# carlamb/MovieRecommender-TF-TRT

Measured on NVIDIA B200. Metric: ncf_train_samples_per_sec, higher is better.
Workload: dtype f32

## Files before the change

movierecommender-tf-trt_b200/csrc/api.cu:

```cuda
#include <math.h>
#include <stdarg.h>
#include <stdlib.h>
#include <string.h>

#include <vector>

#include "launchers.h"
#include "neumf_tile.cuh"

namespace mr {

static thread_local char g_err[512] = "";

void set_error(const char* fmt, ...) {
  va_list ap;
  va_start(ap, fmt);
  vsnprintf(g_err, sizeof(g_err), fmt, ap);
  va_end(ap);
}

int cuda_fail(cudaError_t e, const char* what) {
  set_error("CUDA error in %s: %s", what, cudaGetErrorString(e));
  return MR_ERR_CUDA;
}
// ... 27 lines not shown
};
static thread_local Profiler g_prof;
constexpr size_t kMaxProfEvents = 1 << 16;

void count_launch() { g_prof.launches += 1; }

void prof_mark(int phase, cudaStream_t st) {
  Profiler& p = g_prof;
  if (!p.on) return;
  if (p.used >= kMaxProfEvents) {
    p.overflow = true;
    return;
  }
  if (p.used == p.events.size()) {
    cudaEvent_t e;
    if (cudaEventCreate(&e) != cudaSuccess) {
      cudaGetLastError();
      p.overflow = true;
      return;
    }
    p.events.push_back(e);
    p.phase.push_back(-1);
  }
  cudaEventRecord(p.events[p.used], st);
  p.phase[p.used] = phase;
  p.used += 1;
}

struct SideStream {
  int dev = -1;
  cudaStream_t stream = nullptr;
  cudaEvent_t fork = nullptr, join = nullptr;
  cudaEvent_t fork2 = nullptr, join2 = nullptr;
};
static thread_local SideStream g_side;

static SideStream* side_stream() {
  int dev = 0;
  if (cudaGetDevice(&dev) != cudaSuccess) {
    cudaGetLastError();
    return nullptr;
  }
  SideStream& s = g_side;
  if (s.dev != dev) {
    s = SideStream{};
    if (cudaStreamCreateWithFlags(&s.stream, cudaStreamNonBlocking) != cudaSuccess ||
        cudaEventCreateWithFlags(&s.fork, cudaEventDisableTiming) != cudaSuccess ||
        cudaEventCreateWithFlags(&s.join, cudaEventDisableTiming) != cudaSuccess ||
        cudaEventCreateWithFlags(&s.fork2, cudaEventDisableTiming) != cudaSuccess ||
        cudaEventCreateWithFlags(&s.join2, cudaEventDisableTiming) != cudaSuccess) {
      cudaGetLastError();
      s = SideStream{};
      return nullptr;
    }
    s.dev = dev;
  }
  return &s;
}

__global__ void flag_to_float_kernel(const int32_t* flags, float* out) {
  *out = (float)((flags[0] ? 1 : 0) | (flags[1] ? 2 : 0));
}

static int bits_for(int64_t n) {
  int b = 1;
  while (b < 31 && ((int64_t)1 << b) < n) ++b;
  return b;
}

static int sort_row_ids(const int32_t* ids, int64_t n, int32_t num_rows, int32_t* sorted_keys, int32_t* sorted_index,
                        void* ws, size_t ws_bytes, cudaStream_t st) {
  return launch_sort_pairs(ids, n, bits_for((int64_t)num_rows + 1), sorted_keys, sorted_index, ws, ws_bytes, st,
                           num_rows);
}

static int check_model(const MrModel* m) {
  MR_REQUIRE(m != nullptr, "model is NULL");
  MR_REQUIRE(m->n_layers >= 1 && m->n_layers <= MR_MAX_LAYERS, "n_layers=%d out of [1,%d]", m->n_layers, MR_MAX_LAYERS);
  MR_REQUIRE(m->L[0] >= 2, "layers_sizes[0]=%d must be >= 2", m->L[0]);
  for (int l = 0; l < m->n_layers; ++l)
    MR_REQUIRE(m->L[l] >= 1 && m->L[l] <= MR_MAX_WIDTH, "layers_sizes[%d]=%d out of [1,%d]", l, m->L[l], MR_MAX_WIDTH);
  MR_REQUIRE(m->mf_dim >= 0 && m->mf_dim <= MR_MAX_WIDTH, "mf_dim=%d out of range", m->mf_dim);
  MR_REQUIRE(m->num_users > 0 && m->num_items > 0, "num_users/num_items must be > 0");
// ... 279 lines not shown
  a.K = m.L[0] - d_u;
  a.rows = m.num_items;
  a.row0 = 0;
  a.epilogue = TC_EPI_BIAS_RELU;
  a.linear = true;
  a.out = t.Pi;
  return launch_tc_dense(a, st);
}

static int tc_project_users(const MrModel& m, const TcWs& t, cudaStream_t st) {
  TcDenseArgs a{};
  a.a_dense = m.user_mlp;
  a.b_packed = t.pack_fu;
  a.N = m.L[1];
  a.K = m.L[0] / 2;
  a.rows = m.num_users;
  a.row0 = 0;
  a.epilogue = TC_EPI_BIAS_RELU;
  a.bias = m.b[1];
  a.linear = true;
  a.out = t.Pu;
  return launch_tc_dense(a, st);
}

struct TrainWs {
  int32_t* flags;
  float* wt;
  float* dense_partial;
  int64_t dense_stride;
  float* loss_partial;
  float* probs;
  float* stage_u;
  float* stage_i;
  int32_t* sorted_keys;
  int32_t* sorted_index;
  int32_t* sorted_keys_i;
  int32_t* sorted_index_i;
  void* sort_ws;
  size_t sort_ws_bytes;
  void* seg_ws;
  size_t seg_ws_bytes;
  void* seg_ws_u;
  size_t seg_ws_u_bytes;
  void* tc_ws;
  size_t tc_ws_bytes;
  void* small_ws;
  size_t small_ws_bytes;
  int32_t* pos;
  float* rank_partials;
  int32_t* group_users;
  size_t total;
};

static TrainWs carve_train(const MrModel& m, int64_t B, void* ws) {
  TrainWs t;
  Carver cv(ws);
  const int d_u = m.L[0] / 2, d_i = m.L[0] - d_u;
  const int cap = max_tile_ctas();
  t.flags = cv.take<int32_t>(64);
  t.wt = cv.take<float>(m.dense_count);
  t.dense_stride = (m.dense_count + 3) & ~(int64_t)3;
  t.dense_partial = cv.take<float>((size_t)cap * t.dense_stride);
  t.loss_partial = cv.take<float>(cap);
  t.probs = cv.take<float>(B);
  t.stage_u = cv.take<float>((size_t)B * (d_u + m.mf_dim));
  t.stage_i = cv.take<float>((size_t)B * (d_i + m.mf_dim));
  t.sorted_keys = cv.take<int32_t>(B);
  t.sorted_index = cv.take<int32_t>(B);
  t.sorted_keys_i = cv.take<int32_t>(B);
  t.sorted_index_i = cv.take<int32_t>(B);
  t.sort_ws_bytes = sort_workspace_bytes(B);
  t.sort_ws = cv.take<char>(t.sort_ws_bytes);
  t.seg_ws_bytes = segreduce_workspace_bytes(B, (d_u > d_i ? d_u : d_i) + m.mf_dim);
  t.seg_ws = cv.take<char>(t.seg_ws_bytes);
  t.seg_ws_u_bytes = segreduce_workspace_bytes(B / 2 + 1, d_u + m.mf_dim);
  t.seg_ws_u = cv.take<char>(t.seg_ws_u_bytes);
  t.pos = cv.take<int32_t>(B);
  t.rank_partials = cv.take<float>(rank_partials_count(B));
  t.group_users = cv.take<int32_t>(B / 2 + 1);
  t.tc_ws_bytes = tc_eligible(m) ? carve_tc(m, true, B, nullptr).total : 0;
  t.tc_ws = cv.take<char>(t.tc_ws_bytes);
  t.small_ws_bytes = (!tc_eligible(m) && small_tower_supported(m, 5)) ? carve_small(m, nullptr).total : 0;
  t.small_ws = cv.take<char>(t.small_ws_bytes);
  t.total = cv.off;
  return t;
}

static float adam_lr_t(const MrOptState& o, int64_t t) {
  return (float)((double)o.lr * sqrt(1.0 - pow((double)o.beta_2, (double)t)) / (1.0 - pow((double)o.beta_1, (double)t)));
}

static int check_opt(const MrModel& m, const MrOptState* o, const MrGrads* g) {
  MR_REQUIRE(o != nullptr && g != nullptr, "opt/grads is NULL");
  MR_REQUIRE(o->optimizer == MR_OPT_ADAM || o->optimizer == MR_OPT_SGD, "unknown optimizer %d", o->optimizer);
  MR_REQUIRE(o->table_mode == MR_TABLES_DENSE || o->table_mode == MR_TABLES_SPARSE, "unknown table_mode %d", o->table_mode);
  MR_REQUIRE(g->dense != nullptr, "grads.dense is NULL");
  if (o->optimizer == MR_OPT_ADAM) {
    MR_REQUIRE(o->m_dense && o->v_dense && o->m_user_mlp && o->v_user_mlp && o->m_item_mlp && o->v_item_mlp,
               "Adam state pointers are NULL");
// ... 360 lines not shown
      if (rc == MR_OK) rc = launch_pack_weights(Wu, d_u, m.L[1], 1, tw.pack_bu, st);
      if (rc == MR_OK) rc = launch_pack_weights(Wi, d_i, m.L[1], 1, tw.pack_bi, st);
      if (rc != MR_OK) return rc;
    }
    if (proj) {
      prof_mark(MR_PHASE_TC_DENSE_FWD, st);
      rc = tc_project_items(m, tw, st);
      if (rc == MR_OK && uproj) rc = tc_project_users(m, tw, st);
      if (rc != MR_OK) return rc;
    }
    int fused_grid = 0;
    if (fused) {
      prof_mark(MR_PHASE_FUSED_TILE, st);
      FusedTrainArgs fa{};
      fa.Pi = tw.Pi;
      fa.Pu = tw.Pu;
      fa.user_gmf = m.user_gmf;
      fa.item_gmf = m.item_gmf;
      fa.users = users;
      fa.items = items;
      fa.labels = labels;
      fa.num_users = m.num_users;
      fa.num_items = m.num_items;
      fa.rows = B;
      fa.group = group;
      fa.W2 = m.W[2];
      fa.w2_image = tw.w2_image;
      fa.b2 = m.b[2];
      fa.w_out = m.w_out;
      fa.b_out = m.b_out;
      fa.inv_batch = inv_global_batch;
      fa.probs = t.probs;
      fa.stage_i = t.stage_i;
      fa.stage_u = t.stage_u;
      fa.si = d_i + f;
      fa.su = d_u + f;
      fa.partial = t.dense_partial;
      fa.partial_stride = t.dense_stride;
      fa.off_w2 = m.W[2] - m.dense;
      fa.off_b2 = m.b[2] - m.dense;
      fa.off_wout = m.w_out - m.dense;
      fa.off_bout = m.b_out - m.dense;
      fa.loss_partial = t.loss_partial;
      fa.flags = t.flags;
      rc = launch_fused_train(fa, st, &fused_grid);
      if (rc != MR_OK) return rc;
    }
    const int64_t sb = tc_sub_batch(B);
    for (int64_t r0 = 0; r0 < B && !fused; r0 += sb) {
      const int64_t r1 = r0 + sb < B ? r0 + sb : B;
      prof_mark(MR_PHASE_TC_DENSE_FWD, st);
      rc = tc_forward_rows(m, tw, users, items, 1, r0, r1, st, gdiv);
      if (rc != MR_OK) return rc;
      prof_mark(MR_PHASE_HEAD, st);
      HeadArgs h{};
      h.model = model;
      h.h_last = tw.H[n - 1];
      h.users = users;
      h.items = items;
      h.labels = labels;
      h.rows = r1 - r0;
      h.row0 = r0;
      h.user_div = 1;
      h.group = gdiv;
      h.inv_batch = inv_global_batch;
      h.probs = t.probs;
      h.dz_last = tw.dZ[n - 1];
      h.stage_u = t.stage_u;
// ... 135 lines not shown
          a.si = d_i + f;
        }
        rc = launch_tc_dense(a, st);
        if (rc != MR_OK) return rc;
      }
    }
    if (proj) {
      if (side != nullptr) MR_CUDA(cudaStreamWaitEvent(st, side->join, 0));
      RowUpdate ui{};
      ui.mode = MR_TABLES_DENSE;
      ui.optimizer = opt->optimizer;
      ui.d0 = m.L[1];
      ui.d1 = f;
      ui.num_rows = m.num_items;
      ui.g0 = tw.Si;
      ui.g1 = grads->item_gmf;
      cudaStream_t su_st = st;
      if (uproj && side != nullptr) {
        MR_CUDA(cudaEventRecord(side->fork2, st));
        MR_CUDA(cudaStreamWaitEvent(side->stream, side->fork2, 0));
        su_st = side->stream;
      }
      if (uproj && su_st != st) {
        RowUpdate uu{};
        uu.mode = MR_TABLES_DENSE;
        uu.optimizer = opt->optimizer;
        uu.d0 = m.L[1];
        uu.d1 = f;
        uu.num_rows = m.num_users;
        uu.g0 = tw.Su;
        uu.g1 = grads->user_gmf;
        rc = launch_segreduce(t.sorted_keys, t.sorted_index, n_user_rows, t.stage_u, uu, t.seg_ws_u, t.seg_ws_u_bytes, su_st);
        if (rc != MR_OK) return rc;
        if (grads->user_gmf_ready != nullptr) {
          MR_CUDA(cudaEventRecord((cudaEvent_t)grads->user_gmf_ready, su_st));
          user_gmf_event_recorded = true;
        }
        TcDenseArgs bu{};
        bu.a_dense = tw.Su;
        bu.b_packed = tw.pack_bu;
        bu.N = d_u;
        bu.K = m.L[1];
        bu.rows = m.num_users;
        bu.row0 = 0;
        bu.epilogue = TC_EPI_BIAS_RELU;
        bu.linear = true;
        bu.out = grads->user_mlp;
        rc = launch_tc_dense(bu, su_st);
        if (rc != MR_OK) return rc;
        TcWgradArgs wu{};
        wu.a_dense = m.user_mlp;
        wu.z = tw.Su;
        wu.Fa = d_u;
        wu.Fb = m.L[1];
        wu.rows = m.num_users;
        wu.row0 = 0;
        wu.dw_partial = t.dense_partial + (m.W[1] - m.dense);
        wu.db_partial = t.dense_partial + (m.b[1] - m.dense);
        wu.partial_stride = t.dense_stride;
        rc = launch_tc_wgrad(wu, su_st);
        if (rc != MR_OK) return rc;
        if (grads->user_tables_ready != nullptr) {
          MR_CUDA(cudaEventRecord((cudaEvent_t)grads->user_tables_ready, su_st));
          user_event_recorded = true;
        }
        MR_CUDA(cudaEventRecord(side->join2, su_st));
      }
      prof_mark(MR_PHASE_SEGREDUCE, st);
      rc = launch_segreduce(t.sorted_keys_i, t.sorted_index_i, B, t.stage_i, ui, t.seg_ws, t.seg_ws_bytes, st);
      if (rc != MR_OK) return rc;
      if (uproj && su_st == st) {
        RowUpdate uu{};
        uu.mode = MR_TABLES_DENSE;
        uu.optimizer = opt->optimizer;
        uu.d0 = m.L[1];
        uu.d1 = f;
        uu.num_rows = m.num_users;
        uu.g0 = tw.Su;
        uu.g1 = grads->user_gmf;
        prof_mark(MR_PHASE_SEGREDUCE, st);
        rc = launch_segreduce(t.sorted_keys, t.sorted_index, n_user_rows, t.stage_u, uu, t.seg_ws, t.seg_ws_bytes, st);
        if (rc != MR_OK) return rc;
      }
      prof_mark(MR_PHASE_TC_DENSE_BWD, st);
      TcDenseArgs bi{};
      bi.a_dense = tw.Si;
      bi.b_packed = tw.pack_bi;
      bi.N = d_i;
      bi.K = m.L[1];
      bi.rows = m.num_items;
      bi.row0 = 0;
      bi.epilogue = TC_EPI_BIAS_RELU;
      bi.linear = true;
      bi.out = grads->item_mlp;
      rc = launch_tc_dense(bi, st);
      if (rc != MR_OK) return rc;
      prof_mark(MR_PHASE_TC_WGRAD, st);
      TcWgradArgs wi{};
      wi.a_dense = m.item_mlp;
      wi.z = tw.Si;
      wi.Fa = d_i;
      wi.Fb = m.L[1];
      wi.rows = m.num_items;
// ... 668 lines not shown
```

movierecommender-tf-trt_b200/csrc/launchers.h:

```cpp
#pragma once

#include "common.cuh"

namespace mr {

struct TileLaunch {
  const MrModel* model;
  bool train;
  const float* wt;
  const int32_t* users;
  const int32_t* items;
  const float* labels;
  int64_t B;
  int32_t user_div;
  float inv_batch;
  float* logits;
  float* probs;
  float* loss_partial;
  float* dense_partial;
  int64_t dense_stride;
  float* stage_u;
  float* stage_i;
  int32_t* flags;
};
int max_tile_ctas();
int choose_tile_rows(const MrModel& m, bool train);
int launch_neumf_tiles(const TileLaunch& a, cudaStream_t st, int* grid_out);
int launch_transpose_kernels(const MrModel& m, float* wt, cudaStream_t st);
int launch_dense_reduce(const MrModel& m, const float* partial, int64_t stride, int grid_ctas, float* out,
                        cudaStream_t st, bool with_l2 = true);
int launch_sum_partials(const float* partial, int n, float* out, cudaStream_t st);
int launch_l2_penalty(const float* x, int64_t n, float coef, float* out, cudaStream_t st);

int launch_gather_rows(const float* table, int64_t rows, int dim, const int32_t* idx, int64_t n, float* out,
                       cudaStream_t st);

size_t sort_workspace_bytes(int64_t n);
int launch_sort_pairs(const int32_t* keys, int64_t n, int key_bits, int32_t* out_keys, int32_t* out_index,
                      void* ws, size_t ws_bytes, cudaStream_t st, int32_t num_rows = -1);

struct RowUpdate {
  int mode;
  int optimizer;
  float lr_t, beta_1, beta_2, epsilon, lr;
  int d0, d1;
  int num_rows;
  float *p0, *m0, *v0, *g0;
  float *p1, *m1, *v1, *g1;
};
size_t segreduce_workspace_bytes(int64_t n, int ld);
int launch_segreduce(const int32_t* sorted_keys, const int32_t* sorted_index, int64_t n, const float* staged,
                     const RowUpdate& u, void* ws, size_t ws_bytes, cudaStream_t st);

constexpr int kMaxOptRegions = 5;
struct OptRegions {
  float* p[kMaxOptRegions];
  const float* g[kMaxOptRegions];
  float* m[kMaxOptRegions];
  float* v[kMaxOptRegions];
  int64_t n[kMaxOptRegions];
  float l2[kMaxOptRegions];
  int count;
  int block_start[kMaxOptRegions + 1];
};
int launch_optimizer_regions(OptRegions r, int optimizer, float lr_t, float beta_1, float beta_2, float epsilon,
                             cudaStream_t st);
int launch_optimizer_flat(float* p, const float* g, float* m, float* v, int64_t n, int optimizer, float lr_t,
                          float beta_1, float beta_2, float epsilon, float l2, cudaStream_t st);

size_t rank_partials_count(int64_t G);
int launch_rank_scores(const float* scores, int64_t G, int group, int k, const int32_t* label_col, int32_t* rank,
                       int32_t* pos, float* sums, float* partials, cudaStream_t st, const float* labels = nullptr);

struct TopkArgs {
  const float* scores;
  int64_t U, u0;
  int32_t N, k;
  const int32_t* excl_ids;
  int32_t excl_rows;
  const int64_t* excl_rowptr;
  const int32_t* excl_items;
  const int32_t* targets;
  const int32_t* users;
  int32_t num_users;
  int32_t* top_items;
// ... 139 lines not shown
int launch_group_heads(const int32_t* ids, int64_t groups, int group, int32_t* out, cudaStream_t st);
int launch_check_grouped(const int32_t* ids, int64_t n, int group, int32_t* flag, cudaStream_t st);

size_t split_workspace_bytes(int64_t n);
int launch_split_last_two(const int32_t* users, int64_t n, int32_t num_users, int32_t* order, int32_t* part,
                          int32_t* flag, void* ws, size_t ws_bytes, cudaStream_t st);
size_t remap_workspace_bytes(int64_t n);
int launch_remap_ids(const int32_t* ids, int64_t n, int32_t limit, int32_t* dense, int32_t* unique, int64_t* num_unique,
                     int32_t* flag, void* ws, size_t ws_bytes, cudaStream_t st);
size_t user_csr_workspace_bytes(int64_t n);
int launch_build_user_csr(const int32_t* users, const int32_t* items, int64_t n, int32_t num_users, int32_t num_items,
                          int64_t* rowptr, int32_t* csr_items, int32_t* flag, void* ws, size_t ws_bytes,
                          cudaStream_t st);

struct FusedTrainArgs {
  const float* Pi;
  const float* Pu;
  const float* user_gmf;
  const float* item_gmf;
  const int32_t* users;
  const int32_t* items;
  const float* labels;
  int32_t num_users, num_items;
  int64_t rows;
  int32_t group;
  const float* W2;
  uint16_t* w2_image;
  const float* b2;
  const float* w_out;
  const float* b_out;
  float inv_batch;
  float* probs;
  float* stage_i;
  float* stage_u;
  int32_t si, su;
  float* partial;
  int64_t partial_stride;
  int64_t off_w2, off_b2, off_wout, off_bout;
  float* loss_partial;
  int32_t* flags;
};
bool fused_train_supported(const MrModel& m, int group);
size_t fused_w2_image_bytes();
int launch_fused_train(const FusedTrainArgs& a, cudaStream_t st, int* grid_out);
int launch_bf16x3_selftest(const float* A, const float* B, float* D, int N, int K, int a_mn, int b_mn, cudaStream_t st);

int launch_tc_rate(int N, int iters, int nbuf, int flags, int writers, int write_iters, long long* out, int grid,
                   cudaStream_t st);
int launch_tc_probe(const float* raw_a, int n_words, int start_off, int lbo, int sbo, int a_mn, float* D,
                    cudaStream_t st);
int launch_tc_selftest(const float* A, const float* B, float* D, int N, int K, int a_mn, int b_mn, int three_x,
                       cudaStream_t st);

}
```

movierecommender-tf-trt_b200/csrc/segreduce.cu:

```cuda
#include "launchers.h"

namespace mr {

constexpr int kSkip = -1;
constexpr int kPastEnd = -2;
constexpr int kNoNeighbour = -3;
constexpr int kBatch = 8;
constexpr int kBatchUpper = 16;

__device__ __forceinline__ void apply_row_value(const RowUpdate& u, int row, int c, float g) {
  float *p, *m, *v, *gt;
  int d, col;
  if (c < u.d0) {
    p = u.p0; m = u.m0; v = u.v0; gt = u.g0; d = u.d0; col = c;
  } else {
    p = u.p1; m = u.m1; v = u.v1; gt = u.g1; d = u.d1; col = c - u.d0;
  }
  const size_t at = (size_t)row * d + col;
  if (u.mode == MR_TABLES_DENSE) {
    gt[at] = g;
  } else if (u.optimizer == MR_OPT_ADAM) {
    const float mn = u.beta_1 * m[at] + (1.f - u.beta_1) * g;
    const float vn = u.beta_2 * v[at] + (1.f - u.beta_2) * g * g;
    m[at] = mn;
// ... 14 lines not shown
  }
  const size_t at = (size_t)row * d + col;
  if ((d & 3) != 0) {
    apply_row_value(u, row, c, g.x);
    apply_row_value(u, row, c + 1, g.y);
    apply_row_value(u, row, c + 2, g.z);
    apply_row_value(u, row, c + 3, g.w);
    return;
  }
  if (u.mode == MR_TABLES_DENSE) {
    *reinterpret_cast<float4*>(gt + at) = g;
  } else if (u.optimizer == MR_OPT_ADAM) {
    const float4 m0 = *reinterpret_cast<const float4*>(m + at), v0 = *reinterpret_cast<const float4*>(v + at);
    float4 pw = *reinterpret_cast<const float4*>(p + at);
    float4 mn, vn;
    mn.x = u.beta_1 * m0.x + (1.f - u.beta_1) * g.x; vn.x = u.beta_2 * v0.x + (1.f - u.beta_2) * g.x * g.x;
    mn.y = u.beta_1 * m0.y + (1.f - u.beta_1) * g.y; vn.y = u.beta_2 * v0.y + (1.f - u.beta_2) * g.y * g.y;
    mn.z = u.beta_1 * m0.z + (1.f - u.beta_1) * g.z; vn.z = u.beta_2 * v0.z + (1.f - u.beta_2) * g.z * g.z;
    mn.w = u.beta_1 * m0.w + (1.f - u.beta_1) * g.w; vn.w = u.beta_2 * v0.w + (1.f - u.beta_2) * g.w * g.w;
    pw.x = pw.x - u.lr_t * mn.x / (sqrtf(vn.x) + u.epsilon);
    pw.y = pw.y - u.lr_t * mn.y / (sqrtf(vn.y) + u.epsilon);
    pw.z = pw.z - u.lr_t * mn.z / (sqrtf(vn.z) + u.epsilon);
    pw.w = pw.w - u.lr_t * mn.w / (sqrtf(vn.w) + u.epsilon);
    *reinterpret_cast<float4*>(m + at) = mn;
    *reinterpret_cast<float4*>(v + at) = vn;
    *reinterpret_cast<float4*>(p + at) = pw;
  } else {
    float4 pw = *reinterpret_cast<const float4*>(p + at);
    pw.x -= u.lr * g.x; pw.y -= u.lr * g.y; pw.z -= u.lr * g.z; pw.w -= u.lr * g.w;
    *reinterpret_cast<float4*>(p + at) = pw;
  }
}

struct ChunkInfo {
  int nvalid;
  bool first_inc;
  bool last_inc;
  int64_t chunk;
  int ld;
  float* out_rows;
};

template <bool VEC>
__device__ __forceinline__ void flush_run(const RowUpdate& u, const ChunkInfo& ci, int key, int s, int t, int c,
                                          bool on, float4 acc) {
  if (key == kSkip || !on || (unsigned)key >= (unsigned)u.num_rows) return;
  const bool inc_first = (s == 0) && ci.first_inc;
  const bool inc_last = (t == ci.nvalid) && ci.last_inc;
  if (!inc_first && !inc_last) {
    if (VEC) apply_row_value4(u, key, c, acc);
    else apply_row_value(u, key, c, acc.x);
    return;
  }
  float* slot0 = ci.out_rows + (size_t)(2 * ci.chunk) * ci.ld + c;
  float* slot1 = slot0 + ci.ld;
  if (VEC) {
    if (inc_first) {
      *reinterpret_cast<float4*>(slot0) = acc;
      if (inc_last) *reinterpret_cast<float4*>(slot1) = make_float4(0.f, 0.f, 0.f, 0.f);
    } else {
      *reinterpret_cast<float4*>(slot1) = acc;
    }
  } else {
    if (inc_first) {
      *slot0 = acc.x;
      if (inc_last) *slot1 = 0.f;
    } else {
      *slot1 = acc.x;
    }
  }
}

template <bool INDIRECT, bool VEC, int KB>
__global__ void __launch_bounds__(256) segreduce_level_kernel(const int32_t* __restrict__ keys,
                                                              const int32_t* __restrict__ index, int64_t n,
                                                              const float* __restrict__ rows, int32_t* __restrict__ out_keys,
                                                              float* __restrict__ out_rows, const RowUpdate u) {
  const int lane = threadIdx.x & 31;
  const int64_t chunk = ((int64_t)blockIdx.x * blockDim.x + threadIdx.x) >> 5;
  const int64_t base = chunk * 32;
  if (base >= n) return;
  const int ld = u.d0 + u.d1;
  const int64_t e = base + lane;
  const int key = e < n ? __ldg(keys + e) : kPastEnd;
  const int64_t src = e < n ? (INDIRECT ? (int64_t)__ldg(index + e) : e) : 0;
  const bool ok = e < n && key != kSkip;
  const int kprev = base > 0 ? __ldg(keys + base - 1) : kNoNeighbour;
  const int knext = base + 32 < n ? __ldg(keys + base + 32) : kNoNeighbour;
  int kup = __shfl_up_sync(0xffffffffu, key, 1);
  const unsigned starts = __ballot_sync(0xffffffffu, e < n && (lane == 0 || key != kup));

  ChunkInfo ci;
  ci.nvalid = (int)min((int64_t)32, n - base);
  const int key0 = __shfl_sync(0xffffffffu, key, 0);
  const int keyl = __shfl_sync(0xffffffffu, key, ci.nvalid - 1);
  ci.first_inc = key0 != kSkip && kprev == key0;
  ci.last_inc = ci.nvalid == 32 && keyl != kSkip && knext == keyl;
  ci.chunk = chunk;
  ci.ld = ld;
  ci.out_rows = out_rows;
  if (out_keys != nullptr && lane == 0 && blockIdx.y == 0) {
    out_keys[2 * chunk] = ci.first_inc ? key0 : kSkip;
    out_keys[2 * chunk + 1] = ci.last_inc ? keyl : kSkip;
  }

  constexpr int W = VEC ? 4 : 1;
  for (int cb = blockIdx.y * 32 * W; cb < ld; cb += gridDim.y * 32 * W) {
    const int c = cb + lane * W;
    const bool on = c < ld;
    float4 acc = make_float4(0.f, 0.f, 0.f, 0.f);
    int run_key = key0, run_start = 0;
    for (int j0 = 0; j0 < ci.nvalid; j0 += KB) {
      float4 v[KB];
#pragma unroll
      for (int q = 0; q < KB; ++q) {
        const int j = j0 + q;
        const int64_t sj = __shfl_sync(0xffffffffu, src, j);
        const bool okj = __shfl_sync(0xffffffffu, (int)ok, j) != 0;
        v[q] = make_float4(0.f, 0.f, 0.f, 0.f);
        if (okj && on) {
          if (VEC) v[q] = ld_stream4(rows + (size_t)sj * ld + c);
          else v[q].x = __ldg(rows + (size_t)sj * ld + c);
        }
      }
#pragma unroll
      for (int q = 0; q < KB; ++q) {
        const int j = j0 + q;
        if (j < ci.nvalid) {
          if (j > 0 && ((starts >> j) & 1u)) {
            flush_run<VEC>(u, ci, run_key, run_start, j, c, on, acc);
            acc = make_float4(0.f, 0.f, 0.f, 0.f);
            run_start = j;
            run_key = __shfl_sync(0xffffffffu, key, j);
          }
          acc.x += v[q].x;
          if (VEC) {
            acc.y += v[q].y;
            acc.z += v[q].z;
            acc.w += v[q].w;
          }
        }
      }
    }
    flush_run<VEC>(u, ci, run_key, run_start, ci.nvalid, c, on, acc);
  }
}

static int64_t level_entries(int64_t n) { return 2 * ((n + 31) / 32); }

size_t segreduce_workspace_bytes(int64_t n, int ld) {
  const int64_t n1 = level_entries(n < 1 ? 1 : n), n2 = level_entries(n1);
  return align_up((size_t)n1 * 4, 256) + align_up((size_t)n2 * 4, 256) + align_up((size_t)n1 * ld * 4, 256) +
         align_up((size_t)n2 * ld * 4, 256);
}

int launch_segreduce(const int32_t* sorted_keys, const int32_t* sorted_index, int64_t n, const float* staged,
                     const RowUpdate& u, void* ws, size_t ws_bytes, cudaStream_t st) {
  if (n == 0) return MR_OK;
  const int ld = u.d0 + u.d1;
  if (ws_bytes < segreduce_workspace_bytes(n, ld)) {
    set_error("segreduce workspace too small: %zu < %zu", ws_bytes, segreduce_workspace_bytes(n, ld));
    return MR_ERR_WORKSPACE;
  }
  const int64_t n1 = level_entries(n), n2 = level_entries(n1);
  Carver cv(ws);
  int32_t* kbuf[2] = {cv.take<int32_t>(n1), cv.take<int32_t>(n2)};
  float* rbuf[2] = {cv.take<float>((size_t)n1 * ld), cv.take<float>((size_t)n2 * ld)};
  uintptr_t align = reinterpret_cast<uintptr_t>(staged);
  for (const float* q : {u.p0, u.m0, u.v0, u.g0, u.p1, u.m1, u.v1, u.g1}) align |= reinterpret_cast<uintptr_t>(q);
  const bool vec = (ld & 3) == 0 && (u.d0 & 3) == 0 && (align & 15) == 0;

  const int32_t* keys = sorted_keys;
  const float* rows = staged;
  int64_t cur = n;
  for (int level = 0;; ++level) {
    const int64_t nchunks = (cur + 31) / 32;
    const bool last = nchunks == 1;
    int32_t* ok = last ? nullptr : kbuf[level & 1];
    float* orows = last ? nullptr : rbuf[level & 1];
    const unsigned blocks = (unsigned)((nchunks + 7) / 8);
    if (level == 0) {
      if (vec) segreduce_level_kernel<true, true, kBatch><<<blocks, 256, 0, st>>>(keys, sorted_index, cur, rows, ok, orows, u);
      else segreduce_level_kernel<true, false, kBatch><<<blocks, 256, 0, st>>>(keys, sorted_index, cur, rows, ok, orows, u);
    } else {
      const int per = vec ? 128 : 32;
      const dim3 grid(blocks, (unsigned)((ld + per - 1) / per));
      if (vec) segreduce_level_kernel<false, true, kBatchUpper><<<grid, 256, 0, st>>>(keys, nullptr, cur, rows, ok, orows, u);
      else segreduce_level_kernel<false, false, kBatchUpper><<<grid, 256, 0, st>>>(keys, nullptr, cur, rows, ok, orows, u);
    }
    MR_LAUNCH_CHECK("segreduce_level_kernel");
    if (last) break;
    keys = ok;
    rows = orows;
    cur = 2 * nchunks;
  }
  return MR_OK;
}

}
```

movierecommender-tf-trt_b200/csrc/tc_fused.cu:

```cuda
#include "launchers.h"
#include "tc_bf16x3.cuh"
#include "tc_common.cuh"

namespace mr {
namespace fz {

constexpr int kD1 = 128, kD2 = 64, kF = 64;
constexpr int kThreads = 16 * 32;
constexpr int kProdThreads = 256;
constexpr int kE1Warp0 = 8, kE2Warp0 = 12;
constexpr uint32_t kPanel = 16384;
constexpr uint32_t kH1Part = 2 * kPanel;
constexpr int kEpiLd = 36;

constexpr uint32_t oH1 = 0;
constexpr uint32_t oZ2 = oH1 + 3 * kH1Part;
constexpr uint32_t oW2 = oZ2 + 3 * kPanel;
constexpr uint32_t oStage = oW2 + 3 * kPanel;
constexpr uint32_t oBits = oStage + 4 * 32 * kEpiLd * 4;
constexpr uint32_t oIds = oBits + 2 * 128 * 16;
constexpr uint32_t oGdot = oIds + 2 * 288 * 4;
constexpr uint32_t oDz = oGdot + 512;
constexpr uint32_t oFlag = oDz + 512;
constexpr uint32_t oConst = oFlag + 512;
// ... 23 lines not shown
__device__ __forceinline__ void cp_async_wait_all() { asm volatile("cp.async.wait_all;" ::: "memory"); }
__device__ __forceinline__ void bar_sync(int id, int nthreads) {
  asm volatile("bar.sync %0, %1;" ::"r"(id), "r"(nthreads) : "memory");
}

#ifdef MR_FUSED_TIMING
__device__ long long g_fused_timing[256 * 48];
#define FZ_T_DECL long long tz_[16] = {0}; long long tz_last_ = clock64();
#define FZ_T(seg) { const long long n_ = clock64(); tz_[seg] += n_ - tz_last_; tz_last_ = n_; }
#define FZ_T_FLUSH(role, cond) if (cond) { for (int q_ = 0; q_ < 16; ++q_) g_fused_timing[blockIdx.x * 48 + (role) * 16 + q_] = tz_[q_]; }
#else
#define FZ_T_DECL
#define FZ_T(seg)
#define FZ_T_FLUSH(role, cond)
#endif

struct FusedParams {
  const float* Pi;
  const float* Pu;
  const float* user_gmf;
  const float* item_gmf;
  const int32_t* users;
  const int32_t* items;
  const float* labels;
  int32_t num_users, num_items;
  int64_t rows;
  const uint16_t* w2_image;
  const float* b2;
  const float* w_out;
  const float* b_out;
  float inv_batch;
  float* probs;
  float* stage_i;
  float* stage_u;
  int32_t si, su;
  float* partial;
  int64_t partial_stride;
  int64_t off_w2, off_b2, off_wout, off_bout;
  float* loss_partial;
  int32_t* flags;
};

template <int GROUP>
__global__ void __launch_bounds__(kThreads, 1) neumf_fused_train_kernel(const FusedParams p) {
  constexpr int GQ = 32 / GROUP, RQ = GQ * GROUP, GT = 4 * GQ, TR = 4 * RQ;
  constexpr int NT = GT * 16;
  static_assert((2 * NT) % kProdThreads == 0, "H1 tasks must divide evenly over the producer threads");
  constexpr int SLOTS = 2 * NT / kProdThreads;
  constexpr int GSLOTS = (NT + kProdThreads - 1) / kProdThreads;

  extern __shared__ uint8_t smem_raw[];
  __shared__ uint64_t h1_full[2], fwd_done, gmf_ready, dz2_full, h1_free, bwd_done, e2_done, wg_read, w2_bar;
  __shared__ uint32_t tmem_slot;
  uint8_t* smem = smem_raw + ((1024u - (tc::smem_u32(smem_raw) & 1023u)) & 1023u);

  const int tid = threadIdx.x, warp = tid >> 5, lane = tid & 31;
  const int64_t ntiles = (p.rows + TR - 1) / TR;
  float* gdot_s = reinterpret_cast<float*>(smem + oGdot);
  float* dz_s = reinterpret_cast<float*>(smem + oDz);
  int32_t* flag_s = reinterpret_cast<int32_t*>(smem + oFlag);
  float* const_s = reinterpret_cast<float*>(smem + oConst);

  for (uint32_t e = tid; e < oW2 / 16; e += kThreads) reinterpret_cast<uint4*>(smem)[e] = make_uint4(0u, 0u, 0u, 0u);
  for (int e = tid; e < 128; e += kThreads) {
    gdot_s[e] = 0.f;
    dz_s[e] = 0.f;
// ... 185 lines not shown
      }
      h1_arrive(1);
      FZ_T(4)
      gmf_dot(0, gu[0], gi[0]);
      if (GSLOTS > 1 && g1_live) gmf_dot(1, gu[GSLOTS - 1], gi[GSLOTS - 1]);
      __syncwarp();
      if (lane == 0) tc::mbar_arrive(&gmf_ready);
      FZ_T(5)

      tc::mbar_wait(&dz2_full, (uint32_t)(it & 1));
      FZ_T(6)
#pragma unroll
      for (int s = 0; s < GSLOTS; ++s) {
        const int idx = tidv + kProdThreads * s;
        if (s > 0 && !g1_live) continue;
        const int gt = idx >> 4, pc = idx & 15;
        const int sl0 = 32 * (gt / GQ) + GROUP * (gt % GQ);
        const int64_t grow0 = row0 + (int64_t)gt * GROUP;
        const bool gvalid = grow0 < p.rows;
        float4 ga = make_float4(0.f, 0.f, 0.f, 0.f);
#pragma unroll
        for (int j = 0; j < GROUP; ++j) {
          const float dz = dz_s[sl0 + j];
          const float4 g = make_float4(dz * wg4.x, dz * wg4.y, dz * wg4.z, dz * wg4.w);
          const float4 u4 = gu[s], i4 = gi[s][j];
          accg.x = fmaf(dz, u4.x * i4.x, accg.x);
          accg.y = fmaf(dz, u4.y * i4.y, accg.y);
          accg.z = fmaf(dz, u4.z * i4.z, accg.z);
          accg.w = fmaf(dz, u4.w * i4.w, accg.w);
          ga.x = fmaf(g.x, i4.x, ga.x);
          ga.y = fmaf(g.y, i4.y, ga.y);
          ga.z = fmaf(g.z, i4.z, ga.z);
          ga.w = fmaf(g.w, i4.w, ga.w);
          if (gvalid)
            *reinterpret_cast<float4*>(p.stage_i + (size_t)(grow0 + j) * p.si + kD1 + 4 * pc) =
                make_float4(g.x * u4.x, g.y * u4.y, g.z * u4.z, g.w * u4.w);
        }
        if (gvalid) *reinterpret_cast<float4*>(p.stage_u + (size_t)(grow0 / GROUP) * p.su + kD1 + 4 * pc) = ga;
      }
      FZ_T(7)
      cp_async_wait_all();
      bar_sync(1, kProdThreads);
      FZ_T(8)
    }
    FZ_T_FLUSH(0, tid == 0)
    if (any_bad) atomicOr(p.flags, 1);
    *reinterpret_cast<float4*>(smem + oRedG + 16 * tid) = accg;
  } else if (warp < kE2Warp0) {
    const int quarter = warp & 3;
    const int slot = 32 * quarter + lane;
    const uint32_t lane_addr = tmem_base + ((uint32_t)(32 * quarter) << 16);
    const float b_out = const_s[192];
    const bool issuer = warp == kE1Warp0;
    const uint32_t s0 = tc::smem_u32(smem);
    const uint64_t dk = tc::smem_desc(0, 16, 1024, kLayoutSw128);
    const uint64_t dmn = tc::smem_desc(0, kPanel, 1024, kLayoutSw128);
    const uint32_t id_fwd = idesc_bf16(128, kD2, 0, 1);
    const uint32_t id_bwd = idesc_bf16(128, kD1, 0, 0);
    const uint32_t id_wg = idesc_bf16(128, kD2, 1, 1);
    constexpr int PA[6] = {0, 0, 1, 0, 2, 1}, PB[6] = {0, 1, 0, 2, 0, 1};
    {
      float zero[32];
#pragma unroll
      for (int i = 0; i < 32; ++i) zero[i] = 0.f;
#pragma unroll
      for (int c = 0; c < 4; ++c) tmem_st32(lane_addr + cCs + 32 * c, zero);
    }
    float accb = 0.f, accl = 0.f;
    int64_t it = 0;
    FZ_T_DECL
    for (int64_t tile = blockIdx.x; tile < ntiles; tile += gridDim.x, ++it) {
// ... 293 lines not shown
}

bool fused_train_supported(const MrModel& m, int group) {
  return m.n_layers == 3 && m.L[0] == 2 * fz::kD1 && m.L[1] == fz::kD1 && m.L[2] == fz::kD2 && m.mf_dim == fz::kF && group == 5;
}

size_t fused_w2_image_bytes() { return 3 * fz::kPanel; }

int launch_fused_train(const FusedTrainArgs& a, cudaStream_t st, int* grid_out) {
  if (a.group != 5) {
    set_error("fused train kernel: unsupported group %d", a.group);
    return MR_ERR_INVALID;
  }
  fz::pack_w2_bf16x3_kernel<<<(fz::kD1 * fz::kD2 / 2 + 255) / 256, 256, 0, st>>>(a.W2, a.w2_image);
  MR_LAUNCH_CHECK("pack_w2_bf16x3_kernel");
  fz::FusedParams p{};
  p.Pi = a.Pi;
  p.Pu = a.Pu;
  p.user_gmf = a.user_gmf;
  p.item_gmf = a.item_gmf;
  p.users = a.users;
  p.items = a.items;
  p.labels = a.labels;
  p.num_users = a.num_users;
  p.num_items = a.num_items;
  p.rows = a.rows;
  p.w2_image = a.w2_image;
  p.b2 = a.b2;
  p.w_out = a.w_out;
  p.b_out = a.b_out;
  p.inv_batch = a.inv_batch;
  p.probs = a.probs;
  p.stage_i = a.stage_i;
  p.stage_u = a.stage_u;
  p.si = a.si;
  p.su = a.su;
  p.partial = a.partial;
  p.partial_stride = a.partial_stride;
  p.off_w2 = a.off_w2;
  p.off_b2 = a.off_b2;
  p.off_wout = a.off_wout;
  p.off_bout = a.off_bout;
  p.loss_partial = a.loss_partial;
  p.flags = a.flags;
  constexpr int TR = 4 * (32 / 5) * 5;
  const int64_t ntiles = (a.rows + TR - 1) / TR;
  int64_t grid = sm_count();
  if (grid > ntiles) grid = ntiles;
  if (grid_out) *grid_out = (int)grid;
  if (grid == 0) return MR_OK;
  auto kern = fz::neumf_fused_train_kernel<5>;
  const size_t smem = fz::kSmemBytes + 1024;
  MR_CUDA(cudaFuncSetAttribute(kern, cudaFuncAttributeMaxDynamicSharedMemorySize, (int)smem));
  kern<<<(unsigned)grid, fz::kThreads, smem, st>>>(p);
  MR_LAUNCH_CHECK("neumf_fused_train_kernel");
  return MR_OK;
}

#ifdef MR_FUSED_TIMING
extern "C" int mr_fused_timing_read(long long* out_host) {
  return cudaMemcpyFromSymbol(out_host, fz::g_fused_timing, sizeof(long long) * 256 * 48) == cudaSuccess ? 0 : -1;
}
#endif

}
```

Baseline: 714.2 million.

## Recompute item GMF gradients inside segreduce instead of staging them

The fused train kernel no longer writes the per-row item GMF gradient (dz*w*u) into stage_i. It stores a compact (dz, user id) pair per row, and the first item segreduce level rebuilds the GMF gradient from w_out and the user GMF table, using L2 eviction hints. This cuts global write and read traffic for the staged item rows. The user-side stream now waits for the item reduction before signalling readiness, because the user GMF table must not be updated before it is read, which adds a cross-stream dependency.

```diff
diff --git a/movierecommender-tf-trt_b200/csrc/api.cu b/movierecommender-tf-trt_b200/csrc/api.cu
--- a/movierecommender-tf-trt_b200/csrc/api.cu
+++ b/movierecommender-tf-trt_b200/csrc/api.cu
@@ -83,6 +83,7 @@
   cudaStream_t stream = nullptr;
   cudaEvent_t fork = nullptr, join = nullptr;
   cudaEvent_t fork2 = nullptr, join2 = nullptr;
+  cudaEvent_t items_reduced = nullptr;
 };
 static thread_local SideStream g_side;
 
@@ -99,7 +100,8 @@
         cudaEventCreateWithFlags(&s.fork, cudaEventDisableTiming) != cudaSuccess ||
         cudaEventCreateWithFlags(&s.join, cudaEventDisableTiming) != cudaSuccess ||
         cudaEventCreateWithFlags(&s.fork2, cudaEventDisableTiming) != cudaSuccess ||
-        cudaEventCreateWithFlags(&s.join2, cudaEventDisableTiming) != cudaSuccess) {
+        cudaEventCreateWithFlags(&s.join2, cudaEventDisableTiming) != cudaSuccess ||
+        cudaEventCreateWithFlags(&s.items_reduced, cudaEventDisableTiming) != cudaSuccess) {
       cudaGetLastError();
       s = SideStream{};
       return nullptr;
@@ -445,6 +447,7 @@
   float* probs;
   float* stage_u;
   float* stage_i;
+  int2* dz_user;
   int32_t* sorted_keys;
   int32_t* sorted_index;
   int32_t* sorted_keys_i;
@@ -478,6 +481,7 @@
   t.probs = cv.take<float>(B);
   t.stage_u = cv.take<float>((size_t)B * (d_u + m.mf_dim));
   t.stage_i = cv.take<float>((size_t)B * (d_i + m.mf_dim));
+  t.dz_user = reinterpret_cast<int2*>(t.stage_i + (size_t)B * d_i);
   t.sorted_keys = cv.take<int32_t>(B);
   t.sorted_index = cv.take<int32_t>(B);
   t.sorted_keys_i = cv.take<int32_t>(B);
@@ -904,8 +908,9 @@
       fa.inv_batch = inv_global_batch;
       fa.probs = t.probs;
       fa.stage_i = t.stage_i;
+      fa.dz_user = t.dz_user;
       fa.stage_u = t.stage_u;
-      fa.si = d_i + f;
+      fa.si = d_i;
       fa.su = d_u + f;
       fa.partial = t.dense_partial;
       fa.partial_stride = t.dense_stride;
@@ -1107,7 +1112,7 @@
         uu.g1 = grads->user_gmf;
         rc = launch_segreduce(t.sorted_keys, t.sorted_index, n_user_rows, t.stage_u, uu, t.seg_ws_u, t.seg_ws_u_bytes, su_st);
         if (rc != MR_OK) return rc;
-        if (grads->user_gmf_ready != nullptr) {
+        if (grads->user_gmf_ready != nullptr && !fused) {
           MR_CUDA(cudaEventRecord((cudaEvent_t)grads->user_gmf_ready, su_st));
           user_gmf_event_recorded = true;
         }
@@ -1135,15 +1140,30 @@
         wu.partial_stride = t.dense_stride;
         rc = launch_tc_wgrad(wu, su_st);
         if (rc != MR_OK) return rc;
+        if (grads->user_tables_ready != nullptr && !fused) {
+          MR_CUDA(cudaEventRecord((cudaEvent_t)grads->user_tables_ready, su_st));
+          user_event_recorded = true;
+        }
+        if (!fused) MR_CUDA(cudaEventRecord(side->join2, su_st));
+      }
+      prof_mark(MR_PHASE_SEGREDUCE, st);
+      const StagedGmf sg{t.dz_user, m.w_out, m.user_gmf};
+      rc = launch_segreduce(t.sorted_keys_i, t.sorted_index_i, B, t.stage_i, ui, t.seg_ws, t.seg_ws_bytes, st,
+                            fused ? &sg : nullptr);
+      if (rc != MR_OK) return rc;
+      if (fused && su_st != st) {
+        MR_CUDA(cudaEventRecord(side->items_reduced, st));
+        MR_CUDA(cudaStreamWaitEvent(su_st, side->items_reduced, 0));
+        if (grads->user_gmf_ready != nullptr) {
+          MR_CUDA(cudaEventRecord((cudaEvent_t)grads->user_gmf_ready, su_st));
+          user_gmf_event_recorded = true;
+        }
         if (grads->user_tables_ready != nullptr) {
           MR_CUDA(cudaEventRecord((cudaEvent_t)grads->user_tables_ready, su_st));
           user_event_recorded = true;
         }
         MR_CUDA(cudaEventRecord(side->join2, su_st));
       }
-      prof_mark(MR_PHASE_SEGREDUCE, st);
-      rc = launch_segreduce(t.sorted_keys_i, t.sorted_index_i, B, t.stage_i, ui, t.seg_ws, t.seg_ws_bytes, st);
-      if (rc != MR_OK) return rc;
       if (uproj && su_st == st) {
         RowUpdate uu{};
         uu.mode = MR_TABLES_DENSE;
diff --git a/movierecommender-tf-trt_b200/csrc/launchers.h b/movierecommender-tf-trt_b200/csrc/launchers.h
--- a/movierecommender-tf-trt_b200/csrc/launchers.h
+++ b/movierecommender-tf-trt_b200/csrc/launchers.h
@@ -48,9 +48,14 @@
   float *p0, *m0, *v0, *g0;
   float *p1, *m1, *v1, *g1;
 };
+struct StagedGmf {
+  const int2* dz_user;
+  const float* w;
+  const float* table;
+};
 size_t segreduce_workspace_bytes(int64_t n, int ld);
 int launch_segreduce(const int32_t* sorted_keys, const int32_t* sorted_index, int64_t n, const float* staged,
-                     const RowUpdate& u, void* ws, size_t ws_bytes, cudaStream_t st);
+                     const RowUpdate& u, void* ws, size_t ws_bytes, cudaStream_t st, const StagedGmf* gmf = nullptr);
 
 constexpr int kMaxOptRegions = 5;
 struct OptRegions {
@@ -256,6 +261,7 @@
   float inv_batch;
   float* probs;
   float* stage_i;
+  int2* dz_user;
   float* stage_u;
   int32_t si, su;
   float* partial;
diff --git a/movierecommender-tf-trt_b200/csrc/segreduce.cu b/movierecommender-tf-trt_b200/csrc/segreduce.cu
--- a/movierecommender-tf-trt_b200/csrc/segreduce.cu
+++ b/movierecommender-tf-trt_b200/csrc/segreduce.cu
@@ -70,6 +70,24 @@
   }
 }
 
+__device__ __forceinline__ uint64_t l2_policy_evict_first() {
+  uint64_t pol;
+  asm volatile("createpolicy.fractional.L2::evict_first.b64 %0, 1.0;" : "=l"(pol));
+  return pol;
+}
+__device__ __forceinline__ uint64_t l2_policy_evict_last() {
+  uint64_t pol;
+  asm volatile("createpolicy.fractional.L2::evict_last.b64 %0, 1.0;" : "=l"(pol));
+  return pol;
+}
+__device__ __forceinline__ float4 ld_stream4_policy(const float* p, uint64_t pol) {
+  float4 r;
+  asm volatile("ld.global.nc.L1::no_allocate.L2::cache_hint.v4.f32 {%0, %1, %2, %3}, [%4], %5;"
+               : "=f"(r.x), "=f"(r.y), "=f"(r.z), "=f"(r.w)
+               : "l"(p), "l"(pol));
+  return r;
+}
+
 struct ChunkInfo {
   int nvalid;
   bool first_inc;
@@ -109,20 +127,29 @@
   }
 }
 
-template <bool INDIRECT, bool VEC, int KB>
-__global__ void __launch_bounds__(256) segreduce_level_kernel(const int32_t* __restrict__ keys,
-                                                              const int32_t* __restrict__ index, int64_t n,
-                                                              const float* __restrict__ rows, int32_t* __restrict__ out_keys,
-                                                              float* __restrict__ out_rows, const RowUpdate u) {
+template <bool INDIRECT, bool VEC, int KB, bool GMF>
+__device__ __forceinline__ void segreduce_level(const int32_t* __restrict__ keys, const int32_t* __restrict__ index,
+                                                int64_t n, const float* __restrict__ rows, int32_t* __restrict__ out_keys,
+                                                float* __restrict__ out_rows, const RowUpdate& u, const StagedGmf& g) {
   const int lane = threadIdx.x & 31;
   const int64_t chunk = ((int64_t)blockIdx.x * blockDim.x + threadIdx.x) >> 5;
   const int64_t base = chunk * 32;
   if (base >= n) return;
   const int ld = u.d0 + u.d1;
+  const int rld = GMF ? u.d0 : ld;
   const int64_t e = base + lane;
   const int key = e < n ? __ldg(keys + e) : kPastEnd;
   const int64_t src = e < n ? (INDIRECT ? (int64_t)__ldg(index + e) : e) : 0;
   const bool ok = e < n && key != kSkip;
+  float dz = 0.f;
+  int gu = -1;
+  const uint64_t pol_rows = GMF ? l2_policy_evict_first() : 0;
+  const uint64_t pol_table = GMF ? l2_policy_evict_last() : 0;
+  if (GMF && ok) {
+    const int2 d = __ldg(g.dz_user + src);
+    dz = __int_as_float(d.x);
+    gu = d.y;
+  }
   const int kprev = base > 0 ? __ldg(keys + base - 1) : kNoNeighbour;
   const int knext = base + 32 < n ? __ldg(keys + base + 32) : kNoNeighbour;
   int kup = __shfl_up_sync(0xffffffffu, key, 1);
@@ -146,6 +173,12 @@
   for (int cb = blockIdx.y * 32 * W; cb < ld; cb += gridDim.y * 32 * W) {
     const int c = cb + lane * W;
     const bool on = c < ld;
+    const bool formed = GMF && on && c >= u.d0;
+    float4 w = make_float4(0.f, 0.f, 0.f, 0.f);
+    if (formed) {
+      if (VEC) w = ldg4(g.w + (c - u.d0));
+      else w.x = __ldg(g.w + (c - u.d0));
+    }
     float4 acc = make_float4(0.f, 0.f, 0.f, 0.f);
     int run_key = key0, run_start = 0;
     for (int j0 = 0; j0 < ci.nvalid; j0 += KB) {
@@ -156,14 +189,33 @@
         const int64_t sj = __shfl_sync(0xffffffffu, src, j);
         const bool okj = __shfl_sync(0xffffffffu, (int)ok, j) != 0;
         v[q] = make_float4(0.f, 0.f, 0.f, 0.f);
-        if (okj && on) {
-          if (VEC) v[q] = ld_stream4(rows + (size_t)sj * ld + c);
-          else v[q].x = __ldg(rows + (size_t)sj * ld + c);
+        const int uj = GMF ? __shfl_sync(0xffffffffu, gu, j) : 0;
+        const float* at = rows + (size_t)sj * rld + c;
+        bool load = okj && on;
+        if (GMF && formed) {
+          at = g.table + (size_t)uj * u.d1 + (c - u.d0);
+          load = okj && uj >= 0;
+        }
+        if (load) {
+          if (VEC && GMF) v[q] = ld_stream4_policy(at, formed ? pol_table : pol_rows);
+          else if (VEC) v[q] = ld_stream4(at);
+          else v[q].x = __ldg(at);
         }
       }
 #pragma unroll
       for (int q = 0; q < KB; ++q) {
         const int j = j0 + q;
+        if (GMF) {
+          const float dzj = __shfl_sync(0xffffffffu, dz, j);
+          if (formed) {
+            v[q].x = __fmul_rn(__fmul_rn(dzj, w.x), v[q].x);
+            if (VEC) {
+              v[q].y = __fmul_rn(__fmul_rn(dzj, w.y), v[q].y);
+              v[q].z = __fmul_rn(__fmul_rn(dzj, w.z), v[q].z);
+              v[q].w = __fmul_rn(__fmul_rn(dzj, w.w), v[q].w);
+            }
+          }
+        }
         if (j < ci.nvalid) {
           if (j > 0 && ((starts >> j) & 1u)) {
             flush_run<VEC>(u, ci, run_key, run_start, j, c, on, acc);
@@ -184,6 +236,24 @@
   }
 }
 
+template <bool INDIRECT, bool VEC, int KB>
+__global__ void __launch_bounds__(256) segreduce_level_kernel(const int32_t* __restrict__ keys,
+                                                              const int32_t* __restrict__ index, int64_t n,
+                                                              const float* __restrict__ rows, int32_t* __restrict__ out_keys,
+                                                              float* __restrict__ out_rows, const RowUpdate u) {
+  segreduce_level<INDIRECT, VEC, KB, false>(keys, index, n, rows, out_keys, out_rows, u, StagedGmf{});
+}
+
+template <bool VEC>
+__global__ void __launch_bounds__(256, 3) segreduce_gmf_level_kernel(const int32_t* __restrict__ keys,
+                                                                     const int32_t* __restrict__ index, int64_t n,
+                                                                     const float* __restrict__ rows,
+                                                                     int32_t* __restrict__ out_keys,
+                                                                     float* __restrict__ out_rows, const RowUpdate u,
+                                                                     const StagedGmf g) {
+  segreduce_level<true, VEC, kBatch, true>(keys, index, n, rows, out_keys, out_rows, u, g);
+}
+
 static int64_t level_entries(int64_t n) { return 2 * ((n + 31) / 32); }
 
 size_t segreduce_workspace_bytes(int64_t n, int ld) {
@@ -193,7 +263,7 @@
 }
 
 int launch_segreduce(const int32_t* sorted_keys, const int32_t* sorted_index, int64_t n, const float* staged,
-                     const RowUpdate& u, void* ws, size_t ws_bytes, cudaStream_t st) {
+                     const RowUpdate& u, void* ws, size_t ws_bytes, cudaStream_t st, const StagedGmf* gmf) {
   if (n == 0) return MR_OK;
   const int ld = u.d0 + u.d1;
   if (ws_bytes < segreduce_workspace_bytes(n, ld)) {
@@ -206,7 +276,9 @@
   float* rbuf[2] = {cv.take<float>((size_t)n1 * ld), cv.take<float>((size_t)n2 * ld)};
   uintptr_t align = reinterpret_cast<uintptr_t>(staged);
   for (const float* q : {u.p0, u.m0, u.v0, u.g0, u.p1, u.m1, u.v1, u.g1}) align |= reinterpret_cast<uintptr_t>(q);
+  if (gmf != nullptr) align |= reinterpret_cast<uintptr_t>(gmf->w) | reinterpret_cast<uintptr_t>(gmf->table);
   const bool vec = (ld & 3) == 0 && (u.d0 & 3) == 0 && (align & 15) == 0;
+  const StagedGmf g = gmf != nullptr ? *gmf : StagedGmf{};
 
   const int32_t* keys = sorted_keys;
   const float* rows = staged;
@@ -217,7 +289,10 @@
     int32_t* ok = last ? nullptr : kbuf[level & 1];
     float* orows = last ? nullptr : rbuf[level & 1];
     const unsigned blocks = (unsigned)((nchunks + 7) / 8);
-    if (level == 0) {
+    if (level == 0 && gmf != nullptr) {
+      if (vec) segreduce_gmf_level_kernel<true><<<blocks, 256, 0, st>>>(keys, sorted_index, cur, rows, ok, orows, u, g);
+      else segreduce_gmf_level_kernel<false><<<blocks, 256, 0, st>>>(keys, sorted_index, cur, rows, ok, orows, u, g);
+    } else if (level == 0) {
       if (vec) segreduce_level_kernel<true, true, kBatch><<<blocks, 256, 0, st>>>(keys, sorted_index, cur, rows, ok, orows, u);
       else segreduce_level_kernel<true, false, kBatch><<<blocks, 256, 0, st>>>(keys, sorted_index, cur, rows, ok, orows, u);
     } else {
diff --git a/movierecommender-tf-trt_b200/csrc/tc_fused.cu b/movierecommender-tf-trt_b200/csrc/tc_fused.cu
--- a/movierecommender-tf-trt_b200/csrc/tc_fused.cu
+++ b/movierecommender-tf-trt_b200/csrc/tc_fused.cu
@@ -79,6 +79,7 @@
   float inv_batch;
   float* probs;
   float* stage_i;
+  int2* dz_user;
   float* stage_u;
   int32_t si, su;
   float* partial;
@@ -330,11 +331,12 @@
           ga.y = fmaf(g.y, i4.y, ga.y);
           ga.z = fmaf(g.z, i4.z, ga.z);
           ga.w = fmaf(g.w, i4.w, ga.w);
-          if (gvalid)
-            *reinterpret_cast<float4*>(p.stage_i + (size_t)(grow0 + j) * p.si + kD1 + 4 * pc) =
-                make_float4(g.x * u4.x, g.y * u4.y, g.z * u4.z, g.w * u4.w);
         }
         if (gvalid) *reinterpret_cast<float4*>(p.stage_u + (size_t)(grow0 / GROUP) * p.su + kD1 + 4 * pc) = ga;
+        if (gvalid && pc < GROUP) {
+          const int u = ids[128 + gt];
+          p.dz_user[grow0 + pc] = make_int2(__float_as_int(dz_s[sl0 + pc]), (unsigned)u < (unsigned)p.num_users ? u : -1);
+        }
       }
       FZ_T(7)
       cp_async_wait_all();
@@ -694,6 +696,7 @@
   p.inv_batch = a.inv_batch;
   p.probs = a.probs;
   p.stage_i = a.stage_i;
+  p.dz_user = a.dz_user;
   p.stage_u = a.stage_u;
   p.si = a.si;
   p.su = a.su;
```

After: 720.9 million, median of 6. Within noise of the previous version (+0.9%).
